# KaranSankla/Lidar_Object_Detection

Hardware: AMD Instinct MI355X
Metric: LiDAR points/sec projected+instance-labelled (higher is better)
Workload: dtype f64

## Files before the change

lidar_object_detection_amd/csrc/lpf_cams.hip.h:

```cpp
#pragma once
#include "lpf_kernels.hip.h"

#define LPF_MAX_CAMS_DEV 4

struct LpfCamsArgs {
    LpfParams P[LPF_MAX_CAMS_DEV];
    int C;
    int ntail[LPF_MAX_CAMS_DEV];
};

template <int ROWS, typename LT>
__global__ __launch_bounds__(LPF_BLOCK) void lpf_cams_stream(const LpfCamsArgs A)
{
    __shared__ unsigned s_cnt[LPF_MAX_CAMS_DEV][LPF_TAB_ROWS];
    float4 p[ROWS];
    lpf_k1_tile<ROWS, LPF_K1_FLAGS, LT, false>(A.P[0], (int)blockIdx.x, s_cnt[0], p);
    for (int cam = 1; cam < A.C; ++cam)
        lpf_k1_tile<ROWS, LPF_K1_FLAGS, LT, true>(A.P[cam], (int)blockIdx.x, s_cnt[cam], p);
}

template <bool PRE>
__global__ __launch_bounds__(LPF_BLOCK, 7) void lpf_cams_tail(const LpfCamsArgs A)
{
    __shared__ __attribute__((aligned(16))) char s_raw[LPF_TAIL_LDS];
    const int cam = (int)blockIdx.y;
    if ((int)blockIdx.x >= A.ntail[cam]) return;
    lpf_tail_block<PRE, 1>(A.P[cam], (int)blockIdx.x, s_raw);
}

__global__ __launch_bounds__(LPF_BLOCK) void lpf_cams_finalize(const LpfCamsArgs A)
{
    __shared__ unsigned s_tot[LPF_TAB_ROWS], s_c[LPF_FIN_STAGE];
    const LpfParams &P = A.P[blockIdx.y];
    const int f = (int)blockIdx.x;
    const LpfFrame fr = lpf_frame_record(P.frame0, P.frames, P.F > 1, f);
    lpf_finalize_frame(P, fr, f, s_tot, s_c);
}
```

lidar_object_detection_amd/csrc/lpf_kernels.hip.h:

```cpp
#pragma once
#include <hip/hip_runtime.h>
#include <stdint.h>

#define LPF_BLOCK 256
#define LPF_SEG_QUANTUM 4096
#define LPF_SEG_SMALL 1024
#define LPF_GROUP_SEGS 64
#define LPF_FRM_SHARDS 8
#define LPF_MAX_MASKS_DEV 32
#define LPF_TAB_ROWS 36
#define LPF_TAB_GROUPS 9

struct LpfFrame {
    long long pt_off;
    long long inst_base;
    int N;
    int seg_off;
    int nseg;
    int box_off;
    int B;
    int pad;
    long long cand_off;
    int cand_words;
    int grp_off;
// ... 70 lines not shown
}

__device__ __forceinline__ int lpf_uni(int v) { return __builtin_amdgcn_readfirstlane(v); }
__device__ __forceinline__ long long lpf_uni64(long long v)
{
    return (long long)(((unsigned long long)(unsigned)lpf_uni((int)((unsigned long long)v >> 32)) << 32) | (unsigned)lpf_uni((int)v));
}
__device__ __forceinline__ LpfFrame lpf_frame_record(const LpfFrame &by_value, const LpfFrame *table, const bool many, const int idx)
{
    LpfFrame fr = by_value;
    if (many) {
        const LpfFrame t = table[lpf_uni(idx)];
        fr.pt_off = lpf_uni64(t.pt_off); fr.inst_base = lpf_uni64(t.inst_base); fr.N = lpf_uni(t.N); fr.seg_off = lpf_uni(t.seg_off);
        fr.nseg = lpf_uni(t.nseg); fr.box_off = lpf_uni(t.box_off); fr.B = lpf_uni(t.B); fr.pad = lpf_uni(t.pad);
        fr.cand_off = lpf_uni64(t.cand_off); fr.cand_words = lpf_uni(t.cand_words); fr.grp_off = lpf_uni(t.grp_off); fr.shift = lpf_uni(t.shift);
    }
    return fr;
}

__device__ __forceinline__ int32_t lpf_sat_i32(double r)
{
    int v;
    asm("v_cvt_i32_f64 %0, %1" : "=v"(v) : "v"(r));
    return (r != r) ? INT32_MIN : v;
}

__device__ __forceinline__ unsigned lpf_expo(double x) { return ((unsigned)__double2hiint(x) >> 20) & 0x7ffu; }

__device__ __forceinline__ void lpf_div2(double qx, double qy, double ad, double &uf, double &vf)
{
    const unsigned ea = lpf_expo(ad), ex = lpf_expo(qx), ey = lpf_expo(qy);
    const unsigned lo = min(ea, min(ex, ey)), hi = max(ea, max(ex, ey));
    if (lo >= 723u && hi <= 1323u) {
        double r = __builtin_amdgcn_rcp(ad);
        double e = fma(-ad, r, 1.0); r = fma(r, e, r);
        e = fma(-ad, r, 1.0);        r = fma(r, e, r);
        double q = qx * r; double s = fma(-ad, q, qx); uf = fma(s, r, q);
        q = qy * r;        s = fma(-ad, q, qy);        vf = fma(s, r, q);
    } else {
        uf = qx / ad;
        vf = qy / ad;
    }
}

__device__ __forceinline__ void lpf_project_point(const LpfParams &P, float fx, float fy, float fz,
                                                  double &uf, double &vf, double &d)
{
    const double x = (double)fx, y = (double)fy, z = (double)fz;
    double cx = P.T[0] * x; cx = fma(P.T[1], y, cx); cx = fma(P.T[2],  z, cx); cx = cx + P.T[3];
    double cy = P.T[4] * x; cy = fma(P.T[5], y, cy); cy = fma(P.T[6],  z, cy); cy = cy + P.T[7];
    double cz = P.T[8] * x; cz = fma(P.T[9], y, cz); cz = fma(P.T[10], z, cz); cz = cz + P.T[11];
    double qx = P.K[0] * cx; qx = fma(P.K[1], cy, qx); qx = fma(P.K[2], cz, qx);
    double qy = P.K[3] * cx; qy = fma(P.K[4], cy, qy); qy = fma(P.K[5], cz, qy);
    d = P.K[6] * cx; d = fma(P.K[7], cy, d); d = fma(P.K[8], cz, d);
    if (d == 0.0) d = -1e-6;
    lpf_div2(qx, qy, fabs(d), uf, vf);
}

__device__ __forceinline__ void lpf_project_point_mem(const double *__restrict__ TK, float fx, float fy, float fz,
                                                      double &uf, double &vf, double &d)
{
    const double x = (double)fx, y = (double)fy, z = (double)fz;
    double cx = TK[0] * x; cx = fma(TK[1], y, cx); cx = fma(TK[2],  z, cx); cx = cx + TK[3];
    double cy = TK[4] * x; cy = fma(TK[5], y, cy); cy = fma(TK[6],  z, cy); cy = cy + TK[7];
    double cz = TK[8] * x; cz = fma(TK[9], y, cz); cz = fma(TK[10], z, cz); cz = cz + TK[11];
    double qx = TK[12] * cx; qx = fma(TK[13], cy, qx); qx = fma(TK[14], cz, qx);
    double qy = TK[15] * cx; qy = fma(TK[16], cy, qy); qy = fma(TK[17], cz, qy);
    d = TK[18] * cx; d = fma(TK[19], cy, d); d = fma(TK[20], cz, d);
    if (d == 0.0) d = -1e-6;
    lpf_div2(qx, qy, fabs(d), uf, vf);
}

__device__ __forceinline__ unsigned lpf_f32_to_u8(float v)
{
    int t;
    if (!(v > -2147483904.0f && v < 2147483648.0f)) t = INT32_MIN; else t = (int)v;
    return (unsigned)t & 0xFFu;
}

template <typename T, int MODE>
__device__ __forceinline__ bool lpf_member(T v)
{
    if (MODE == 0) return v != 0;
    if (MODE == 1) return lpf_f32_to_u8((float)v) != 0u;
    if (MODE == 3) return (float)v > 0.5f;
    return lpf_f32_to_u8((float)v * 255.0f) == 255u;
}

template <typename T, int MODE> struct LpfDirect { };
template <typename LT> struct LpfIsDirect { static constexpr bool value = false; };
template <typename T, int MODE> struct LpfIsDirect<LpfDirect<T, MODE> > { static constexpr bool value = true; };

template <typename T, int MODE> struct LpfDirectRect { };
template <typename LT> struct LpfIsDirectRect { static constexpr bool value = false; };
template <typename T, int MODE> struct LpfIsDirectRect<LpfDirectRect<T, MODE> > { static constexpr bool value = true; };
template <typename T, int MODE> struct LpfIsDirect<LpfDirectRect<T, MODE> > { static constexpr bool value = true; };

template <typename LT>
struct LpfLabelSrc {
    typedef LT elem;
    static __device__ __forceinline__ uint32_t get(const elem *__restrict__ img, const LpfParams &, const int pix, const int4 *, int, int) { return (uint32_t)img[pix]; }
    static __device__ __forceinline__ size_t frame_stride(const LpfParams &P) { return (size_t)P.W * (size_t)P.H; }
};
template <typename T, int MODE>
struct LpfLabelSrc<LpfDirect<T, MODE> > {
    typedef T elem;
    static __device__ __forceinline__ uint32_t get(const elem *__restrict__ msk, const LpfParams &P, const int pix, const int4 *__restrict__ rc,
                                                   const int ui, const int vi)
    {
        const size_t hw = (size_t)P.W * (size_t)P.H;
        uint32_t l = 0;
        for (int m0 = 0; m0 < P.M; m0 += 8) {
            T v[8];
#pragma unroll
            for (int j = 0; j < 8; ++j) v[j] = msk[(size_t)min(m0 + j, P.M - 1) * hw + pix];
#pragma unroll
            for (int j = 0; j < 8; ++j)
                if (m0 + j < P.M && lpf_member<T, MODE>(v[j])) l |= 1u << (m0 + j);
        }
        if (rc && l) {
            uint32_t rest = l;
            while (rest) {
                const int m = __ffs(rest) - 1;
                rest &= rest - 1u;
                const int4 q = rc[m];
                if (!(ui >= q.x && ui < q.z && vi >= q.y && vi < q.w)) l &= ~(1u << m);
            }
        }
        return l;
    }
    static __device__ __forceinline__ size_t frame_stride(const LpfParams &P) { return (size_t)P.M * (size_t)P.W * (size_t)P.H; }
};

template <typename T, int MODE>
struct LpfLabelSrc<LpfDirectRect<T, MODE> > {
    typedef T elem;
    static constexpr int mode = MODE;
    static __device__ __forceinline__ uint32_t get(const elem *__restrict__, const LpfParams &, const int, const int4 *, int, int) { return 0u; }
    static __device__ __forceinline__ size_t frame_stride(const LpfParams &P) { return (size_t)P.M * (size_t)P.W * (size_t)P.H; }
};

#define LPF_F_X4 1u
#define LPF_F_NTLOAD 2u
#define LPF_F_NTSTORE 4u
#define LPF_F_LAB_NOMATH 8u
#define LPF_F_LAB_NOGATHER 16u
#define LPF_F_LAB_NOSTORE 32u

#define LPF_F_LAB_NOBAL 64u
#define LPF_F_LAB_NOTAB 128u

#define LPF_RG_SHIFT 4
#define LPF_RG_CELL (1 << LPF_RG_SHIFT)
__device__ __forceinline__ unsigned lpf_wave_or(unsigned x);

template <int ROWS, unsigned FL, typename LT, bool PRELOADED>
__device__ __forceinline__ void lpf_k1_tile(const LpfParams &P, const int blk, unsigned *s_cnt, float4 (&p)[ROWS])
{
    constexpr int TILE = LPF_BLOCK * ROWS;
    static_assert(LPF_SEG_QUANTUM % TILE == 0 && (LPF_SEG_SMALL % TILE == 0 || ROWS >= 8), "tiles must divide segments (8-row and larger tiles: large geometry only)");
    const int tid = threadIdx.x, lane = lpf_lane(), wave = lpf_wave();
    const int tiles_per_seg = P.seg_pts / TILE;
    const int lb = lpf_xcd_remap(blk, P.nseg_total * tiles_per_seg);
    const int sid = lb / tiles_per_seg;
    LpfFrame fr = P.frame0;
    if (P.F > 1) fr = P.segs[__builtin_amdgcn_readfirstlane(sid)];
    const int f = fr.pad;
    const int sh = fr.shift;
    const long long pbase = fr.pt_off - sh;
    const int seg_start = (sid - fr.seg_off) * P.seg_pts;
    const int seg_end = min(seg_start + P.seg_pts, fr.N + sh);
    const int c = seg_start + (lb - sid * tiles_per_seg) * TILE;
    if (c >= seg_end) return;
    const float4 *__restrict__ pts = P.pts + pbase;
    typedef LpfLabelSrc<LT> Src;
    const typename Src::elem *__restrict__ limg =
        (P.label_img && P.M > 0) ? static_cast<const typename Src::elem *>(P.label_img) + (size_t)f * Src::frame_stride(P) : nullptr;
    const int rows_per_seg = P.seg_pts >> 6;
    if (tid < LPF_TAB_ROWS) s_cnt[tid] = 0;
    __syncthreads();
    unsigned nvalid_w = 0, nmask_w = 0;

    {
        const int wbase = c + wave * (ROWS * 64) + lane;
#pragma unroll
        for (int r = 0; r < ROWS; ++r) {
            if constexpr (PRELOADED) continue;
            const float4 *src = pts + min(wbase + r * 64, seg_end - 1);
            if (FL & LPF_F_NTLOAD) {
                typedef float f4v __attribute__((ext_vector_type(4)));
                const f4v t = __builtin_nontemporal_load(reinterpret_cast<const f4v *>(src));
                p[r] = make_float4(t.x, t.y, t.z, t.w);
            } else {
                p[r] = *src;
            }
        }
        uint32_t lab[ROWS];
        bool valid[ROWS];
        constexpr bool RECT = LpfIsDirectRect<LT>::value;
        const int4 *__restrict__ rc_f = ((RECT || LpfIsDirect<LT>::value) && P.rects) ? P.rects + (size_t)f * P.M : nullptr;
        const uint32_t *__restrict__ rgrid = (RECT && limg && P.rect_grid) ? P.rect_grid + (size_t)f * P.rg_cells : nullptr;
        const size_t mhw = (size_t)P.W * (size_t)P.H;
        unsigned long long myv = 0, mym = 0;
        auto consume = [&](const int r, uint32_t l, const bool okr) {
            const int idx = wbase + r * 64;
            if (idx >= sh && idx < seg_end && P.label_bits && !(FL & LPF_F_LAB_NOSTORE)) {
                if (FL & LPF_F_NTSTORE) __builtin_nontemporal_store(l, P.label_bits + pbase + idx);
                else P.label_bits[pbase + idx] = l;
            }
            const unsigned long long vb = __ballot(okr);
            const unsigned long long mb = __ballot(l != 0);
            if (lane == r) { myv = vb; mym = mb; }
            if (l && P.mlist && !(FL & LPF_F_LAB_NOSTORE))
                P.mlist[pbase + (wbase - lane) + ((wbase - lane) == 0 ? sh : 0) + nmask_w + __popcll(mb & ((1ull << lane) - 1ull))] =
                    make_float4(p[r].x, p[r].y, p[r].z, __uint_as_float(l));
            nvalid_w += __popcll(vb);
            nmask_w += __popcll(mb);
            while (l) {
                const int m = __ffs(l) - 1;
                l &= l - 1;
                atomicAdd(&s_cnt[2 + m], 1u);
            }
        };
#pragma unroll
        for (int r = 0; r < ROWS; ++r) {
            const int idx = wbase + r * 64;
            const bool live = idx >= sh && idx < seg_end;
            if (FL & LPF_F_X4) asm volatile("" ::"v"(p[r].w));
            double uf, vf, d, ru, rv;
            if (FL & LPF_F_LAB_NOMATH) {
                uf = (double)p[r].x; vf = (double)p[r].y; d = (double)p[r].z;
                ru = uf + 700.0; rv = vf + 100.0;
            } else {
                lpf_project_point(P, p[r].x, p[r].y, p[r].z, uf, vf, d);
                ru = rint(uf); rv = rint(vf);
            }
            const int ui = lpf_sat_i32(ru), vi = lpf_sat_i32(rv);
            const bool ok = live && ((unsigned)ui < (unsigned)P.W) && ((unsigned)vi < (unsigned)P.H) &&
                            (d > P.dmin) && (d < P.dmax);
            valid[r] = ok;
            lab[r] = 0;
            if constexpr (RECT) {
                if (ok && rgrid) lab[r] = rgrid[(vi >> LPF_RG_SHIFT) * P.rg_cw + (ui >> LPF_RG_SHIFT)];
            } else
            if (!(FL & LPF_F_LAB_NOGATHER)) {
                if (ok && limg) lab[r] = Src::get(limg, P, vi * P.W + ui, rc_f, ui, vi);
            }
            if (live && !(FL & LPF_F_LAB_NOSTORE)) {
                const long long g = pbase + idx;
                if (P.uv) {
                    if (FL & LPF_F_NTSTORE) {
                        typedef int i2v __attribute__((ext_vector_type(2)));
                        i2v t; t.x = ui; t.y = vi;
                        __builtin_nontemporal_store(t, reinterpret_cast<i2v *>(P.uv + g));
                    } else {
                        P.uv[g] = make_int2(ui, vi);
                    }
                }
                if (P.depth) P.depth[g] = d;
                if (P.uf) P.uf[g] = uf;
                if (P.vf) P.vf[g] = vf;
            }
        }
#pragma unroll
        for (int r = 0; r < ROWS; ++r) {
            uint32_t l = lab[r];
            if constexpr (RECT) {
                if (__any(l != 0u)) {
                    double uf, vf, d;
                    lpf_project_point(P, p[r].x, p[r].y, p[r].z, uf, vf, d);
                    const int ui = lpf_sat_i32(rint(uf)), vi = lpf_sat_i32(rint(vf));
                    const unsigned pix = (unsigned)(vi * P.W + ui);
                    uint32_t any = lpf_wave_or(l), l2 = 0u;
                    while (any) {
                        const int m = __ffs(any) - 1;
                        any &= any - 1u;
                        const int4 q = rc_f[m];
                        const bool in = ((l >> m) & 1u) && ui >= q.x && ui < q.z && vi >= q.y && vi < q.w;
                        if (__any(in)) {
                            const typename Src::elem *__restrict__ mk = limg + (size_t)m * mhw;
                            if (in && lpf_member<typename Src::elem, Src::mode>(mk[pix])) l2 |= 1u << m;
                        }
                    }
                    l = l2;
                }
            }
            consume(r, l, valid[r]);
        }
        if (lane < ROWS && !(FL & LPF_F_LAB_NOBAL)) {
            const size_t row = (size_t)sid * rows_per_seg + ((c - seg_start) >> 6) + wave * ROWS + lane;
            P.vbal[row] = myv;
            P.mbal[row] = mym;
        }
    }
    if (lane == 0) { atomicAdd(&s_cnt[0], nvalid_w); atomicAdd(&s_cnt[1], nmask_w); }
    __syncthreads();
    if (!(FL & LPF_F_LAB_NOTAB)) {
        if (tid < (2 + P.M + 1) >> 1) {
            const unsigned long long v = (unsigned long long)s_cnt[2 * tid] | ((unsigned long long)s_cnt[2 * tid + 1] << 32);
            if (v) {
                int seg_off = P.frame0.seg_off, grp_off = P.frame0.grp_off, fid = P.frame0.pad;
                if (P.F > 1) { const LpfFrame *e = P.segs + lpf_uni(sid); seg_off = e->seg_off; grp_off = e->grp_off; fid = e->pad; }
                const int k = sid - seg_off, g = tid >> 1, h = tid & 1;
                atomicAdd(reinterpret_cast<unsigned long long *>(P.seg_tab + (size_t)g * P.nseg_cap + sid) + h, v);
                atomicAdd(reinterpret_cast<unsigned long long *>(P.grp_tab + (size_t)g * P.ngrp_cap + grp_off + (k >> 6)) + h, v);
                atomicAdd(reinterpret_cast<unsigned long long *>(P.frm_tab + ((size_t)fid * LPF_FRM_SHARDS + (k & (LPF_FRM_SHARDS - 1))) * LPF_TAB_GROUPS + g) + h, v);
            }
        }
    }
}

template <int ROWS, unsigned FL, typename LT>
__device__ __forceinline__ void lpf_k1_tile(const LpfParams &P, const int blk, unsigned *s_cnt)
{
    float4 p[ROWS];
    lpf_k1_tile<ROWS, FL, LT, false>(P, blk, s_cnt, p);
}

template <int ROWS, unsigned FL, typename LT = uint32_t>
__global__ __launch_bounds__(LPF_BLOCK) void lpf_k1_project_t(const LpfParams P)
{
    __shared__ unsigned s_cnt[LPF_TAB_ROWS];
    lpf_k1_tile<ROWS, FL, LT>(P, (int)blockIdx.x, s_cnt);
}

#define LPF_K1_FLAGS (LPF_F_X4 | LPF_F_NTLOAD | LPF_F_NTSTORE)

__device__ __forceinline__ bool lpf_oriented_inside(double px, double py, double pz, const double *__restrict__ b)
{
    const double rx = px - b[0], ry = py - b[1], rz = pz - b[2];
    const bool exact_ok = b[15] != 0.0;
#pragma unroll
    for (int a = 0; a < 3; ++a) {
        const double v0 = b[3 + 4 * a], v1 = b[4 + 4 * a], v2 = b[5 + 4 * a], vv = b[6 + 4 * a];
        double d = v1 * ry; d = fma(v0, rx, d); d = fma(v2, rz, d);
        bool in;
        if (exact_ok && !(fabs(d) < 1e-200 && d != 0.0)) {
            in = (d >= 0.0) && (d <= vv);
        } else {
            const double t = d / vv;
            in = (t >= 0.0) && (t <= 1.0);
        }
        if (!in) return false;
    }
    return true;
}

__device__ __forceinline__ bool lpf_aabb_inside(double px, double py, double pz, const double *__restrict__ b)
{
    return (px >= b[0]) && (px <= b[3]) && (py >= b[1]) && (py <= b[4]) && (pz >= b[2]) && (pz <= b[5]);
}

__device__ __forceinline__ unsigned lpf_rl(unsigned v, int l) { return (unsigned)__builtin_amdgcn_readlane((int)v, l); }
__device__ __forceinline__ float lpf_rlf(float v, int l) { return __int_as_float(__builtin_amdgcn_readlane(__float_as_int(v), l)); }
__device__ __forceinline__ unsigned long long lpf_rl64(unsigned long long v, int l)
{
    return (unsigned long long)lpf_rl((unsigned)v, l) | ((unsigned long long)lpf_rl((unsigned)(v >> 32), l) << 32);
}
#define LPF_DPP_ADD(x, ctrl, rows) ((x) + (unsigned)__builtin_amdgcn_update_dpp(0, (int)(x), (ctrl), (rows), 0xf, false))
__device__ __forceinline__ unsigned lpf_wave_sum(unsigned x)
{
    x = LPF_DPP_ADD(x, 0xB1, 0xf);
    x = LPF_DPP_ADD(x, 0x4E, 0xf);
    x = LPF_DPP_ADD(x, 0x141, 0xf);
    x = LPF_DPP_ADD(x, 0x140, 0xf);
    x = LPF_DPP_ADD(x, 0x142, 0xa);
    x = LPF_DPP_ADD(x, 0x143, 0xc);
    return lpf_rl(x, 63);
}
__device__ __forceinline__ unsigned lpf_sum8(unsigned x)
{
    x = LPF_DPP_ADD(x, 0xB1, 0xf);
    x = LPF_DPP_ADD(x, 0x4E, 0xf);
    x = LPF_DPP_ADD(x, 0x141, 0xf);
    return lpf_rl(x, 0);
}
__device__ __forceinline__ unsigned lpf_wave_or(unsigned x)
{
#define LPF_DPP_OR(x, ctrl, rows) ((x) | (unsigned)__builtin_amdgcn_update_dpp(0, (int)(x), (ctrl), (rows), 0xf, false))
    x = LPF_DPP_OR(x, 0xB1, 0xf); x = LPF_DPP_OR(x, 0x4E, 0xf); x = LPF_DPP_OR(x, 0x141, 0xf); x = LPF_DPP_OR(x, 0x140, 0xf);
    x = LPF_DPP_OR(x, 0x142, 0xa); x = LPF_DPP_OR(x, 0x143, 0xc);
#undef LPF_DPP_OR
    return lpf_rl(x, 63);
}

__device__ __forceinline__ void lpf_block_excl4(const unsigned sum[4], unsigned excl[4], unsigned all[4],
                                                unsigned (*s_wsum)[4], int lane, int wave)
{
    unsigned inc[4];
#pragma unroll
    for (int j = 0; j < 4; ++j) {
        unsigned x = sum[j];
#pragma unroll
        for (int o = 1; o < 64; o <<= 1) {
            const unsigned t = __shfl_up(x, o);
            if (lane >= o) x += t;
        }
        inc[j] = x;
        if (lane == 63) s_wsum[wave][j] = x;
    }
    __syncthreads();
#pragma unroll
    for (int j = 0; j < 4; ++j) {
        unsigned wo = 0, a = 0;
#pragma unroll
        for (int w = 0; w < 4; ++w) { const unsigned t = s_wsum[w][j]; if (w < wave) wo += t; a += t; }
        excl[j] = wo + inc[j] - sum[j];
        all[j] = a;
    }
    __syncthreads();
}

__global__ __launch_bounds__(LPF_BLOCK) void lpf_scan_segments(const LpfParams P)
{
    __shared__ unsigned s_toff[LPF_TAB_GROUPS][LPF_BLOCK][4];
    __shared__ unsigned s_wsum[4][4], s_tot[LPF_TAB_ROWS], s_off[LPF_TAB_ROWS];
    const int f = blockIdx.x, tid = threadIdx.x, lane = lpf_lane(), wave = lpf_wave();
    const LpfFrame fr = lpf_frame_record(P.frame0, P.frames, P.F > 1, f);
    const int seg_lo = fr.seg_off, seg_hi = fr.seg_off + fr.nseg;
    const int ngroups = (2 + P.M + 3) >> 2;
    const int R = (fr.nseg + LPF_BLOCK - 1) / LPF_BLOCK;
    const int my_lo = min(seg_lo + tid * R, seg_hi), my_hi = min(my_lo + R, seg_hi);
    for (int g = 0; g < ngroups; ++g) {
        const uint4 *__restrict__ row = P.seg_tab + (size_t)g * P.nseg_cap;
        unsigned sum[4] = {0, 0, 0, 0};
#pragma unroll 8
        for (int sg = my_lo; sg < my_hi; ++sg) {
            const uint4 v = row[sg];
            sum[0] += v.x; sum[1] += v.y; sum[2] += v.z; sum[3] += v.w;
        }
        unsigned excl[4], all[4];
        lpf_block_excl4(sum, excl, all, s_wsum, lane, wave);
#pragma unroll
        for (int j = 0; j < 4; ++j) { s_toff[g][tid][j] = excl[j]; if (tid == 0) s_tot[4 * g + j] = all[j]; }
    }
    __syncthreads();
    if (tid < LPF_TAB_ROWS) {
        const bool used = tid < 4 * ngroups;
        unsigned off = 0;
        if (used) for (int c = 2; c < tid; ++c) off += s_tot[c];
        s_off[tid] = off;
    }
    __syncthreads();
    for (int g = 0; g < ngroups; ++g) {
        const uint4 *__restrict__ row = P.seg_tab + (size_t)g * P.nseg_cap;
        uint4 *__restrict__ pre = P.seg_pre + (size_t)g * P.nseg_cap;
        unsigned run[4];
#pragma unroll
        for (int j = 0; j < 4; ++j) run[j] = s_off[4 * g + j] + s_toff[g][tid][j];
#pragma unroll 8
        for (int sg = my_lo; sg < my_hi; ++sg) {
            const uint4 v = row[sg];
            pre[sg] = make_uint4(run[0], run[1], run[2], run[3]);
            run[0] += v.x; run[1] += v.y; run[2] += v.z; run[3] += v.w;
        }
    }
}

#define LPF_LISTS_WAVES 4
#define LPF_LIST_CAP 1024


__device__ __forceinline__ void lpf_bits_to_list(unsigned long long rowbits, unsigned rowbase, int lane, unsigned short *lst)
{
    unsigned pos = rowbase;
    const unsigned short tag = (unsigned short)(lane * 64);
    while (rowbits) {
        const int b = __ffsll((long long)rowbits) - 1;
        rowbits &= rowbits - 1ull;
        lst[pos++] = (unsigned short)(tag + b);
    }
}

template <bool PRE, int STEP>
__device__ __forceinline__ void lpf_list_prefix(const LpfParams &P, const LpfFrame &fr, const int sid, unsigned &bef, unsigned &tot)
{
// ... 669 lines not shown

__global__ __launch_bounds__(LPF_BLOCK) void lpf_finalize(const LpfParams P)
{
    __shared__ unsigned s_tot[LPF_TAB_ROWS], s_c[LPF_FIN_STAGE];
    const int f = blockIdx.x;
    const LpfFrame fr = lpf_frame_record(P.frame0, P.frames, P.F > 1, f);
    lpf_finalize_frame(P, fr, f, s_tot, s_c);
}

struct LpfStepLayout {
    int nfin, nfin8;
    int nbox, nbox8;
    int ntail;
    int kper, nper;
    int nk1;
    int nrg, nrg8;
    int npack;
    int rest;
#ifdef LPF_LAB
    unsigned long long *clk;
#endif
};
#ifdef LPF_LAB
#define LPF_ROLE_BEGIN const unsigned long long t0_ = wall_clock64();
#define LPF_ROLE_END(role)                                                                                              \
    if (Y.clk) {                                                                                                        \
        __syncthreads();                                                                                                \
        if (threadIdx.x == 0) {                                                                                         \
            const unsigned long long t1_ = wall_clock64();                                                              \
            unsigned long long *k_ = Y.clk + 5 * (role);                                                                \
            atomicMin(k_, t0_); atomicMax(k_ + 1, t1_); atomicAdd(k_ + 2, t1_ - t0_); atomicAdd(k_ + 3, 1ull);          \
            atomicMax(k_ + 4, t1_ - t0_);                                                                               \
        }                                                                                                               \
    }
#else
#define LPF_ROLE_BEGIN
#define LPF_ROLE_END(role)
#endif
struct LpfBoxFrame {
    int box_off, B;
    long long cand_off;
};
struct LpfBoxJob {
    const double *src;
    const uint8_t *enabled_in;
    int cam0, filter_visible, oriented, F;
    double Tcv[12];
    double K[9];
    int W, H, chunks;
    const LpfBoxFrame *bframes;
    LpfBoxFrame frame0;
    double *boxp; float *boxq; unsigned long long *cand;
    double *corners_keep;
    uint8_t *enabled_out;
    uint8_t *visible; double *corners_out; double *bbox2d; int32_t *front;
};
struct LpfBoxJobLds {
    double c[32][8][3];
    unsigned long long grid[LPF_GRID_CELLS];
    float bnd[64][4];
    float dom[4];
};

__device__ __forceinline__ void lpf_box_frame_block(const LpfBoxJob &J, const int blk, char *s_raw);
struct LpfPackJob {
    const uint8_t *masks;
    void *label;
    long long hw, total16;
    int M, W;
    const int4 *rects;
};
template <typename T, int MODE, typename LT>
__device__ __forceinline__ void lpf_pack16_block(const T *__restrict__ masks, LT *__restrict__ label,
                                                 const int M, const long long hw, const long long total16, const long long blk,
                                                 const int4 *__restrict__ rects, const int W);

struct LpfRectJob {
    const int4 *rects;
    uint32_t *grid;
    int F, M, cw, ch, cells, bpf;
};
__device__ __forceinline__ void lpf_rect_grid_block(const LpfRectJob &G, const int blk)
{
    const int f = blk / G.bpf, i = (blk - f * G.bpf) * LPF_BLOCK + (int)threadIdx.x;
    if (f >= G.F || i >= G.cells) return;
    const int cy = i / G.cw, cx = i - cy * G.cw;
    const int x0 = cx << LPF_RG_SHIFT, y0 = cy << LPF_RG_SHIFT;
    const int4 *__restrict__ rc = G.rects + (size_t)lpf_uni(f) * G.M;
    uint32_t bits = 0u;
    for (int m0 = 0; m0 < G.M; m0 += 8) {
        int4 q[8];
#pragma unroll
        for (int j = 0; j < 8; ++j) q[j] = rc[min(m0 + j, G.M - 1)];
#pragma unroll
        for (int j = 0; j < 8; ++j)
            if (m0 + j < G.M && q[j].x < x0 + LPF_RG_CELL && q[j].z > x0 && q[j].y < y0 + LPF_RG_CELL && q[j].w > y0 && q[j].z > q[j].x && q[j].w > q[j].y)
                bits |= 1u << (m0 + j);
    }
    G.grid[(size_t)f * G.cells + i] = bits;
}
__global__ __launch_bounds__(LPF_BLOCK) void lpf_rect_grid_kernel(const LpfRectJob G) { lpf_rect_grid_block(G, (int)blockIdx.x); }

template <int ROWS, unsigned FL, typename LT, bool PRE, bool BOXES>
__global__ __launch_bounds__(LPF_BLOCK, 7) void lpf_step_t(const LpfParams P, const LpfParams Q, const LpfParams R, const LpfStepLayout Y,
                                                           const LpfPackJob J, const LpfBoxJob X, const LpfRectJob G)
{
    __shared__ __attribute__((aligned(16))) char s_raw[LPF_STEP_LDS];
    __shared__ unsigned s_cnt[LPF_TAB_ROWS];
    int b = (int)blockIdx.x;
    LPF_ROLE_BEGIN
    if (b < Y.nfin8) {
        if (b < Y.nfin) {
            const LpfFrame fr = lpf_frame_record(R.frame0, R.frames, R.F > 1, b);
            lpf_finalize_frame(R, fr, b, s_cnt, reinterpret_cast<unsigned *>(s_raw));
            LPF_ROLE_END(0)
        }
        return;
    }
    b -= Y.nfin8;
    if (b < Y.nbox8) {
        if constexpr (BOXES) {
            if (b < Y.nbox) { lpf_box_frame_block(X, b, s_raw); LPF_ROLE_END(1) }
        }
        return;
    }
    b -= Y.nbox8;
    if (b < Y.nrg8) {
        if (b < Y.nrg) lpf_rect_grid_block(G, b);
        return;
    }
    b -= Y.nrg8;
    const int plen = Y.kper + 8, periodic = Y.nper * plen;
    int vblk;
    if (b < periodic) {
        const int per = b / plen, pos = b - per * plen;
        if (pos >= Y.kper) {
            const int tb = per * 8 + (pos - Y.kper);
            if (tb < Y.ntail) { lpf_tail_block<PRE, 2>(Q, tb, s_raw); LPF_ROLE_END(tb < (Q.count_boxes ? Q.ncblk : 0) ? 3 : 2) }
            return;
        }
        vblk = ((per * (Y.kper >> 3) + (pos >> 3)) << 3) | (pos & 7);
    } else {
        const int r = b - periodic;
        if (r >= Y.rest) {
            if constexpr (!LpfIsDirect<LT>::value) {
                if (r - Y.rest < Y.npack) { lpf_pack16_block<uint8_t, 0, LT>(J.masks, static_cast<LT *>(J.label), J.M, J.hw, J.total16, r - Y.rest, J.rects, J.W); LPF_ROLE_END(4) }
            }
            return;
        }
        vblk = ((Y.nper * (Y.kper >> 3) + (r >> 3)) << 3) | (r & 7);
    }
    const int x = vblk & 7, q = Y.nk1 >> 3, rem = Y.nk1 & 7;
    if ((vblk >> 3) >= q + (x < rem ? 1 : 0)) return;
    lpf_k1_tile<ROWS, FL, LT>(P, vblk, s_cnt);
    LPF_ROLE_END(5)
}

__global__ __launch_bounds__(LPF_BLOCK) void lpf_resize_linear_u8_kernel(const uint8_t *__restrict__ src, uint8_t *__restrict__ dst,
                                                                         const int4 *__restrict__ xtab, const int4 *__restrict__ ytab,
                                                                         const int w, const int h, const int W, const int H, const long long total)
{
    const long long i = (long long)blockIdx.x * LPF_BLOCK + threadIdx.x;
    if (i >= total) return;
    const long long hw = (long long)W * H;
    const long long n = i / hw;
    const int rem = (int)(i - n * hw), y = rem / W, x = rem - y * W;
    const int4 cx = xtab[x], cy = ytab[y];
    const uint8_t *__restrict__ s = src + (size_t)n * w * h;
    const int r0 = cy.x * w, r1 = cy.y * w;
    const int S0 = (int)s[r0 + cx.x] * cx.z + (int)s[r0 + cx.y] * cx.w;
    const int S1 = (int)s[r1 + cx.x] * cx.z + (int)s[r1 + cx.y] * cx.w;
    dst[i] = (uint8_t)((((cy.z * (S0 >> 4)) >> 16) + ((cy.w * (S1 >> 4)) >> 16) + 2) >> 2);
}

#define LPF_R2H_BLOCKS 8
struct LpfToHost {
    long long *valid_idx; int2 *uv_valid; uint32_t *label_valid; long long *inst_idx; int32_t *count_mb; void *summary;
    long long inst_cap;
    int n_count;
};

__global__ __launch_bounds__(LPF_BLOCK) void lpf_results_to_host(const LpfParams P, const LpfToHost D)
{
    const int f = (int)blockIdx.x / LPF_R2H_BLOCKS, part = (int)blockIdx.x - f * LPF_R2H_BLOCKS;
    if (f >= P.F) return;
    const LpfFrame fr = lpf_frame_record(P.frame0, P.frames, P.F > 1, f);
    const long long *S = reinterpret_cast<const long long *>(static_cast<const char *>(P.summary) + (size_t)f * LPF_SUMMARY_BYTES);
    const long long nv = S[0];
    long long tot = S[34 + LPF_MAX_MASKS_DEV];
    if (tot > D.inst_cap) tot = D.inst_cap;
    const long long t0 = (long long)part * LPF_BLOCK + threadIdx.x, step = (long long)LPF_R2H_BLOCKS * LPF_BLOCK;
    const long long a = fr.pt_off;
    if (D.valid_idx) for (long long i = t0; i < nv; i += step) D.valid_idx[a + i] = P.valid_idx[a + i];
    if (D.uv_valid) for (long long i = t0; i < nv; i += step) D.uv_valid[a + i] = P.uv_valid[a + i];
    if (D.label_valid) for (long long i = t0; i < nv; i += step) D.label_valid[a + i] = P.label_valid[a + i];
    if (D.inst_idx) {
        const long long b = (long long)f * D.inst_cap;
        for (long long i = t0; i < tot; i += step) D.inst_idx[b + i] = P.inst_idx[b + i];
    }
    if (part == 0) {
        long long *dst = reinterpret_cast<long long *>(static_cast<char *>(D.summary) + (size_t)f * LPF_SUMMARY_BYTES);
        for (int i = threadIdx.x; i < LPF_SUMMARY_BYTES / 8; i += LPF_BLOCK) dst[i] = S[i];
    }
    if (D.count_mb)
        for (long long i = (long long)blockIdx.x * LPF_BLOCK + threadIdx.x; i < D.n_count; i += (long long)gridDim.x * LPF_BLOCK) D.count_mb[i] = P.count_out[i];
}

__global__ __launch_bounds__(LPF_BLOCK) void lpf_resize_area2_u8_kernel(const uint8_t *__restrict__ src, uint8_t *__restrict__ dst,
                                                                        const int W, const int H, const long long quads)
{
    const long long i = (long long)blockIdx.x * LPF_BLOCK + threadIdx.x;
    if (i >= quads) return;
    const int qw = (W + 3) >> 2;
    const long long row = i / qw;
    const int x0 = (int)(i - row * qw) * 4, nx = min(4, W - x0);
    const uint8_t *__restrict__ s0 = src + (size_t)row * 4 * W + 2 * x0;
    const uint8_t *__restrict__ s1 = s0 + 2 * W;
    uint8_t *__restrict__ d = dst + (size_t)row * W + x0;
    for (int k = 0; k < nx; ++k)
        d[k] = (uint8_t)(((int)s0[2 * k] + (int)s0[2 * k + 1] + (int)s1[2 * k] + (int)s1[2 * k + 1] + 2) >> 2);
}

__global__ __launch_bounds__(LPF_BLOCK) void lpf_erode_u8_kernel(const uint8_t *__restrict__ src, uint8_t *__restrict__ dst, const int w, const int h,
                                                                 const long long total)
{
    const long long i = (long long)blockIdx.x * LPF_BLOCK + threadIdx.x;
    if (i >= total) return;
    const long long hw = (long long)w * h;
    const long long rem = i % hw;
    const int y = (int)(rem / w), x = (int)(rem - (long long)y * w);
    unsigned v = src[i];
    if (x > 0) v = min(v, (unsigned)src[i - 1]);
    if (x + 1 < w) v = min(v, (unsigned)src[i + 1]);
    if (y > 0) v = min(v, (unsigned)src[i - w]);
    if (y + 1 < h) v = min(v, (unsigned)src[i + w]);
    dst[i] = (uint8_t)v;
}

__global__ __launch_bounds__(LPF_BLOCK) void lpf_points_in_boxes_kernel(const float *__restrict__ pts, long long k, int stride,
                                                                        const double *__restrict__ boxp, int B, int oriented,
                                                                        uint8_t *__restrict__ inside)
{
    __shared__ double s_box[32][16];
    const long long i = (long long)blockIdx.x * LPF_BLOCK + threadIdx.x;
    double px = 0, py = 0, pz = 0;
    if (i < k) { px = (double)pts[i * stride]; py = (double)pts[i * stride + 1]; pz = (double)pts[i * stride + 2]; }
    for (int b0 = 0; b0 < B; b0 += 32) {
        const int nb = min(32, B - b0);
        __syncthreads();
        for (int j = threadIdx.x; j < nb * 16; j += LPF_BLOCK) s_box[j >> 4][j & 15] = boxp[(size_t)b0 * 16 + j];
        __syncthreads();
        if (i < k)
            for (int b = 0; b < nb; ++b)
                inside[(size_t)(b0 + b) * k + i] =
                    (uint8_t)(oriented ? lpf_oriented_inside(px, py, pz, s_box[b]) : lpf_aabb_inside(px, py, pz, s_box[b]));
    }
}

template <int PASS>
__global__ __launch_bounds__(LPF_BLOCK) void lpf_depth_image_kernel(const LpfParams P, int n, unsigned *__restrict__ win,
                                                                    double *__restrict__ D)
{
    const int i = blockIdx.x * LPF_BLOCK + threadIdx.x;
    if (i >= n) return;
    const float4 p = P.pts[i];
    double uf, vf, d;
    lpf_project_point(P, p.x, p.y, p.z, uf, vf, d);
    const int ui = lpf_sat_i32(rint(uf)), vi = lpf_sat_i32(rint(vf));
    if (((unsigned)ui < (unsigned)P.W) && ((unsigned)vi < (unsigned)P.H) && (d > P.dmin) && (d < P.dmax)) {
        const size_t pix = (size_t)vi * P.W + ui;
        if (PASS == 0) atomicMax(&win[pix], (unsigned)i + 1u);
        else if (win[pix] == (unsigned)i + 1u) D[pix] = d;
    }
}

struct LpfBoxPrep { double Tcv[16]; double K[9]; int W, H; };

__global__ __launch_bounds__(LPF_BLOCK) void lpf_box_prep_kernel(const LpfBoxPrep A, const double *__restrict__ corners_cam, int nbox,
                                                                 uint8_t *__restrict__ visible, double *__restrict__ corners_velo,
                                                                 double *__restrict__ bbox2d, int *__restrict__ front)
{
    const double *Tcv = A.Tcv, *K = A.K;
    const int W = A.W, H = A.H;
    const int t = blockIdx.x * LPF_BLOCK + threadIdx.x;
    const int b = t >> 3, k = t & 7;
    const bool live = b < nbox;
    double x = 0, y = 0, z = 0;
    if (live) { const double *c = corners_cam + ((size_t)b * 8 + k) * 3; x = c[0]; y = c[1]; z = c[2]; }
    double qx = K[0] * x; qx = fma(K[1], y, qx); qx = fma(K[2], z, qx);
    double qy = K[3] * x; qy = fma(K[4], y, qy); qy = fma(K[5], z, qy);
    double d  = K[6] * x; d  = fma(K[7], y, d);  d  = fma(K[8], z, d);
    if (d == 0.0) d = -1e-6;
    const double ad = fabs(d);
    const double ru = rint(qx / ad), rv = rint(qy / ad);
    const bool in_img = (ru >= 0.0) && (ru < (double)W) && (rv >= 0.0) && (rv < (double)H);
    const bool vis = live && (d > 0.1) && in_img;
    const bool fr = live && (d > 0.0);
    const unsigned long long grp = 0xFFull << (lpf_lane() & 56);
    const int nvis = __popcll(__ballot(vis) & grp), nfront = __popcll(__ballot(fr) & grp);
    double umin = fr ? ru : 1e300, umax = fr ? ru : -1e300, vmin = fr ? rv : 1e300, vmax = fr ? rv : -1e300;
#pragma unroll
    for (int o = 1; o < 8; o <<= 1) {
        umin = fmin(umin, __shfl_xor(umin, o)); umax = fmax(umax, __shfl_xor(umax, o));
        vmin = fmin(vmin, __shfl_xor(vmin, o)); vmax = fmax(vmax, __shfl_xor(vmax, o));
    }
    if (live) {
        double *o = corners_velo + ((size_t)b * 8 + k) * 3;
// ... 406 lines not shown
```

Before: 173.1 billion.

## Cache rects in LDS, prefetch first mask bytes, aggregate per-mask counts by ballot

```diff
diff --git a/lidar_object_detection_amd/csrc/lpf_cams.hip.h b/lidar_object_detection_amd/csrc/lpf_cams.hip.h
--- a/lidar_object_detection_amd/csrc/lpf_cams.hip.h
+++ b/lidar_object_detection_amd/csrc/lpf_cams.hip.h
@@ -13,10 +13,11 @@
 __global__ __launch_bounds__(LPF_BLOCK) void lpf_cams_stream(const LpfCamsArgs A)
 {
     __shared__ unsigned s_cnt[LPF_MAX_CAMS_DEV][LPF_TAB_ROWS];
+    __shared__ int4 s_rc[LpfIsDirectRect<LT>::value ? LPF_RECT_MAX : 1];
     float4 p[ROWS];
-    lpf_k1_tile<ROWS, LPF_K1_FLAGS, LT, false>(A.P[0], (int)blockIdx.x, s_cnt[0], p);
+    lpf_k1_tile<ROWS, LPF_K1_FLAGS, LT, false>(A.P[0], (int)blockIdx.x, s_cnt[0], s_rc, p);
     for (int cam = 1; cam < A.C; ++cam)
-        lpf_k1_tile<ROWS, LPF_K1_FLAGS, LT, true>(A.P[cam], (int)blockIdx.x, s_cnt[cam], p);
+        lpf_k1_tile<ROWS, LPF_K1_FLAGS, LT, true>(A.P[cam], (int)blockIdx.x, s_cnt[cam], s_rc, p);
 }
 
 template <bool PRE>
diff --git a/lidar_object_detection_amd/csrc/lpf_kernels.hip.h b/lidar_object_detection_amd/csrc/lpf_kernels.hip.h
--- a/lidar_object_detection_amd/csrc/lpf_kernels.hip.h
+++ b/lidar_object_detection_amd/csrc/lpf_kernels.hip.h
@@ -246,10 +246,17 @@
 
 #define LPF_RG_SHIFT 4
 #define LPF_RG_CELL (1 << LPF_RG_SHIFT)
+#define LPF_RECT_MAX 32
+#ifndef LPF_RECT_K
+#define LPF_RECT_K 2
+#endif
+#ifndef LPF_RECT_KEEP_UV
+#define LPF_RECT_KEEP_UV 1
+#endif
 __device__ __forceinline__ unsigned lpf_wave_or(unsigned x);
 
 template <int ROWS, unsigned FL, typename LT, bool PRELOADED>
-__device__ __forceinline__ void lpf_k1_tile(const LpfParams &P, const int blk, unsigned *s_cnt, float4 (&p)[ROWS])
+__device__ __forceinline__ void lpf_k1_tile(const LpfParams &P, const int blk, unsigned *s_cnt, int4 *s_rc, float4 (&p)[ROWS])
 {
     constexpr int TILE = LPF_BLOCK * ROWS;
     static_assert(LPF_SEG_QUANTUM % TILE == 0 && (LPF_SEG_SMALL % TILE == 0 || ROWS >= 8), "tiles must divide segments (8-row and larger tiles: large geometry only)");
@@ -272,6 +279,10 @@
         (P.label_img && P.M > 0) ? static_cast<const typename Src::elem *>(P.label_img) + (size_t)f * Src::frame_stride(P) : nullptr;
     const int rows_per_seg = P.seg_pts >> 6;
     if (tid < LPF_TAB_ROWS) s_cnt[tid] = 0;
+    constexpr bool RECT = LpfIsDirectRect<LT>::value;
+    if constexpr (RECT) {
+        if (P.rects && tid < min(P.M, LPF_RECT_MAX)) s_rc[tid] = P.rects[(size_t)f * P.M + tid];
+    }
     __syncthreads();
     unsigned nvalid_w = 0, nmask_w = 0;
 
@@ -291,9 +302,10 @@
         }
         uint32_t lab[ROWS];
         bool valid[ROWS];
-        constexpr bool RECT = LpfIsDirectRect<LT>::value;
-        const int4 *__restrict__ rc_f = ((RECT || LpfIsDirect<LT>::value) && P.rects) ? P.rects + (size_t)f * P.M : nullptr;
-        const uint32_t *__restrict__ rgrid = (RECT && limg && P.rect_grid) ? P.rect_grid + (size_t)f * P.rg_cells : nullptr;
+        constexpr bool KEEP_UV = RECT && LPF_RECT_KEEP_UV;
+        int ku[KEEP_UV ? ROWS : 1], kv[KEEP_UV ? ROWS : 1];
+        const int4 *__restrict__ rc_f = (!RECT && LpfIsDirect<LT>::value && P.rects) ? P.rects + (size_t)f * P.M : nullptr;
+        const uint32_t *__restrict__ rgrid = (RECT && limg && P.rect_grid && P.rects) ? P.rect_grid + (size_t)f * P.rg_cells : nullptr;
         const size_t mhw = (size_t)P.W * (size_t)P.H;
         unsigned long long myv = 0, mym = 0;
         auto consume = [&](const int r, uint32_t l, const bool okr) {
@@ -310,10 +322,14 @@
                     make_float4(p[r].x, p[r].y, p[r].z, __uint_as_float(l));
             nvalid_w += __popcll(vb);
             nmask_w += __popcll(mb);
-            while (l) {
-                const int m = __ffs(l) - 1;
-                l &= l - 1;
-                atomicAdd(&s_cnt[2 + m], 1u);
+            if (mb) {
+                uint32_t any = lpf_wave_or(l);
+                while (any) {
+                    const int m = __ffs(any) - 1;
+                    any &= any - 1u;
+                    const unsigned n = (unsigned)__popcll(__ballot((l >> m) & 1u));
+                    if (lane == 0) atomicAdd(&s_cnt[2 + m], n);
+                }
             }
         };
 #pragma unroll
@@ -336,6 +352,7 @@
             lab[r] = 0;
             if constexpr (RECT) {
                 if (ok && rgrid) lab[r] = rgrid[(vi >> LPF_RG_SHIFT) * P.rg_cw + (ui >> LPF_RG_SHIFT)];
+                if constexpr (KEEP_UV) { ku[r] = ui; kv[r] = vi; }
             } else
             if (!(FL & LPF_F_LAB_NOGATHER)) {
                 if (ok && limg) lab[r] = Src::get(limg, P, vi * P.W + ui, rc_f, ui, vi);
@@ -356,24 +373,69 @@
                 if (P.vf) P.vf[g] = vf;
             }
         }
+        constexpr int RK = RECT ? LPF_RECT_K : 1;
+        typedef typename Src::elem Elem;
+        Elem mv[RECT ? ROWS : 1][RK];
+        (void)mv; (void)ku; (void)kv;
+        auto row_pixel = [&](const int r, int &ui, int &vi) {
+            if constexpr (KEEP_UV) { ui = ku[r]; vi = kv[r]; }
+            else {
+                double uf, vf, d;
+                lpf_project_point(P, p[r].x, p[r].y, p[r].z, uf, vf, d);
+                ui = lpf_sat_i32(rint(uf)); vi = lpf_sat_i32(rint(vf));
+            }
+        };
+        if constexpr (RECT) {
+#pragma unroll
+            for (int r = 0; r < ROWS; ++r) {
+#pragma unroll
+                for (int k = 0; k < RK; ++k) mv[r][k] = Elem(0);
+                if (__any(lab[r] != 0u)) {
+                    int ui, vi;
+                    row_pixel(r, ui, vi);
+                    const unsigned pix = (unsigned)(vi * P.W + ui);
+                    uint32_t rest = lab[r];
+                    int m[RK];
+                    int4 q[RK];
+                    bool in[RK];
+#pragma unroll
+                    for (int k = 0; k < RK; ++k) {
+                        in[k] = rest != 0u;
+                        m[k] = in[k] ? __ffs(rest) - 1 : 0;
+                        q[k] = s_rc[m[k]];
+                        rest &= rest - 1u;
+                    }
+#pragma unroll
+                    for (int k = 0; k < RK; ++k)
+                        if (in[k] && ui >= q[k].x && ui < q[k].z && vi >= q[k].y && vi < q[k].w) mv[r][k] = limg[(size_t)m[k] * mhw + pix];
+                }
+            }
+        }
 #pragma unroll
         for (int r = 0; r < ROWS; ++r) {
             uint32_t l = lab[r];
             if constexpr (RECT) {
                 if (__any(l != 0u)) {
-                    double uf, vf, d;
-                    lpf_project_point(P, p[r].x, p[r].y, p[r].z, uf, vf, d);
-                    const int ui = lpf_sat_i32(rint(uf)), vi = lpf_sat_i32(rint(vf));
-                    const unsigned pix = (unsigned)(vi * P.W + ui);
-                    uint32_t any = lpf_wave_or(l), l2 = 0u;
-                    while (any) {
-                        const int m = __ffs(any) - 1;
-                        any &= any - 1u;
-                        const int4 q = rc_f[m];
-                        const bool in = ((l >> m) & 1u) && ui >= q.x && ui < q.z && vi >= q.y && vi < q.w;
-                        if (__any(in)) {
-                            const typename Src::elem *__restrict__ mk = limg + (size_t)m * mhw;
-                            if (in && lpf_member<typename Src::elem, Src::mode>(mk[pix])) l2 |= 1u << m;
+                    uint32_t rest = l, l2 = 0u;
+#pragma unroll
+                    for (int k = 0; k < RK; ++k) {
+                        if (lpf_member<Elem, Src::mode>(mv[r][k])) l2 |= rest & (0u - rest);
+                        rest &= rest - 1u;
+                    }
+                    if (__any(rest != 0u)) {
+                        int ui, vi;
+                        row_pixel(r, ui, vi);
+                        const unsigned pix = (unsigned)(vi * P.W + ui);
+                        uint32_t any = lpf_wave_or(rest);
+                        while (any) {
+                            const int m = __ffs(any) - 1;
+                            any &= any - 1u;
+                            const int4 q = s_rc[m];
+                            const bool in = ((rest >> m) & 1u) && ui >= q.x && ui < q.z && vi >= q.y && vi < q.w;
+                            if (__any(in)) {
+                                const Elem *__restrict__ mk = limg + (size_t)m * mhw;
+                                if (in && lpf_member<Elem, Src::mode>(mk[pix])) l2 |= 1u << m;
+                            }
                         }
                     }
                     l = l2;
@@ -405,17 +467,18 @@
 }
 
 template <int ROWS, unsigned FL, typename LT>
-__device__ __forceinline__ void lpf_k1_tile(const LpfParams &P, const int blk, unsigned *s_cnt)
+__device__ __forceinline__ void lpf_k1_tile(const LpfParams &P, const int blk, unsigned *s_cnt, int4 *s_rc)
 {
     float4 p[ROWS];
-    lpf_k1_tile<ROWS, FL, LT, false>(P, blk, s_cnt, p);
+    lpf_k1_tile<ROWS, FL, LT, false>(P, blk, s_cnt, s_rc, p);
 }
 
 template <int ROWS, unsigned FL, typename LT = uint32_t>
 __global__ __launch_bounds__(LPF_BLOCK) void lpf_k1_project_t(const LpfParams P)
 {
     __shared__ unsigned s_cnt[LPF_TAB_ROWS];
-    lpf_k1_tile<ROWS, FL, LT>(P, (int)blockIdx.x, s_cnt);
+    __shared__ int4 s_rc[LpfIsDirectRect<LT>::value ? LPF_RECT_MAX : 1];
+    lpf_k1_tile<ROWS, FL, LT>(P, (int)blockIdx.x, s_cnt, s_rc);
 }
 
 #define LPF_K1_FLAGS (LPF_F_X4 | LPF_F_NTLOAD | LPF_F_NTSTORE)
@@ -1391,7 +1454,7 @@
     }
     const int x = vblk & 7, q = Y.nk1 >> 3, rem = Y.nk1 & 7;
     if ((vblk >> 3) >= q + (x < rem ? 1 : 0)) return;
-    lpf_k1_tile<ROWS, FL, LT>(P, vblk, s_cnt);
+    lpf_k1_tile<ROWS, FL, LT>(P, vblk, s_cnt, reinterpret_cast<int4 *>(s_raw));
     LPF_ROLE_END(5)
 }
 
```

Result: slower. 169.1 billion (-2.3%).
